# PrayagS/Seriation-in-Paleontological-Data-using-MCMC

Measured on AMD Instinct MI355X. Metric: chain-iterations/sec (100 chains, 256x512 matrix) at 1/2/4/8 MI355X, higher is better.
Workload: dtype f64

## Files before the change

### __graft_entry__.py

```python
import os
import subprocess
import sys

ROOT = os.path.dirname(os.path.abspath(__file__))
PKG = os.path.join(ROOT, "seriation-in-paleontological-data-using-mcmc_amd")


def _paths():
    for p in (PKG, os.path.join(ROOT, "tests")):
        if p not in sys.path:
            sys.path.insert(0, p)


def prewarm(test_shapes=True):
    from concurrent.futures import ThreadPoolExecutor
    _paths()
    import seriation_amd as sa
    ddir = os.path.join(ROOT, "tests", "golden", "datasets")
    paths = sorted(os.path.join(ddir, f) for f in os.listdir(ddir) if f.endswith(".txt"))

    def soft(what, fn):
        try:
            return fn()
        except sa.SrError as e:
            print("prewarm: %s skipped (%s)" % (what, e), file=sys.stderr)
            return 0

    def one(p):
        return soft(os.path.basename(p), lambda: sa.specialize(sa.Dataset.load(p, maxs=0)))

    import numpy as np

    def shape(t):
        N, M, nh, tb = t
        hard = np.zeros(N, np.uint8)
        hard[:nh] = 1
        return soft("shape %r" % (t,), lambda: sa.specialize(sa.Dataset(np.zeros((N, M), np.uint8), hard),
                                                            block_threads=tb))

    shapes = []
    if test_shapes:
        try:
            import spec_shapes
            shapes = spec_shapes.shapes()
            import test_gpu_logl_walk
            import test_gpu_sweep_tail
            shapes = sorted(set(shapes) | set(test_gpu_logl_walk.lds_shapes()) | set(test_gpu_sweep_tail.lds_shapes()))
        except ImportError:
            pass
    with ThreadPoolExecutor(max_workers=min(8, os.cpu_count() or 1)) as ex:
        out = dict(zip([os.path.basename(p) for p in paths], ex.map(one, paths)))
        out["test shapes"] = sum(bool(r) for r in ex.map(shape, shapes))
    return out


def build():
    jobs = str(min(16, os.cpu_count() or 1))
    subprocess.check_call(["make", "-s", "-j" + jobs, "-C", PKG])
    subprocess.check_call(["make", "-s", "-j" + jobs, "-C", os.path.join(ROOT, "oracle")])
    _paths()
    import seriation_amd
    seriation_amd.lib()
    prewarm()


def smoke():
    _paths()
    import numpy as np
    import oracle_ref
    import seriation_amd as sa

    if sa.lib().sr_device_count() <= 0:
        raise RuntimeError("smoke: no gfx950 device visible")
    with open(os.path.join(ROOT, "tests", "golden", "datasets", "g10s10.txt"), "rb") as fh:
        text = fh.read()
    ds = sa.Dataset.parse(text)
    seeds = [1, 2]
    summ, (ri, rd) = sa.run_chains(ds, seeds, burnin_calls=1, sample_calls=3, keep_records=True, device=0)
    for k, s in enumerate(seeds):
        o = oracle_ref.run_chain(text, s, 1, 3)
# ... 12 lines not shown
```

### include/seriation.h

```cpp
#ifndef SERIATION_H
#define SERIATION_H
#include <stddef.h>
#include <stdint.h>
#ifdef __cplusplus
extern "C" {
#endif

#define SR_OK 0
#define SR_EINVAL (-1)
#define SR_EPARSE (-2)
#define SR_EHEADER (-3)
#define SR_ENOMEM (-4)
#define SR_EDEVICE (-5)
#define SR_EUNSUPPORTED (-6)
#define SR_EIO (-7)
#define SR_EINCONSISTENT (-8)

#define SR_MAXS 2000

typedef struct {
  int32_t N, M, nh;
  uint8_t *X;
  uint8_t *hard;
} sr_dataset;
// ... 229 lines not shown
  int64_t *dist, *dist_mirror;
  int64_t scale;
  double kernel_ms;
} sr_agree_out;

int sr_agreement(const sr_dataset *ds, const int16_t *ab_pi, int32_t n_sel, int32_t count, int32_t device,
                 sr_agree_out *out);
int sr_session_agreement(sr_session *s, const int32_t *chains, int32_t n_sel, int32_t first, int32_t count,
                         sr_agree_out *out);
int sr_agreement_distances(int32_t N, int32_t n_sel, const uint32_t *pair_counts, int32_t device, int64_t *dist,
                           int64_t *dist_mirror, double *kernel_ms);
int sr_agreement_modes(int32_t n, const int64_t *dist, const int64_t *dist_mirror, int64_t scale, double threshold,
                       int32_t *mode, uint8_t *flip, int32_t *medoid, int32_t *size, int32_t *n_modes);

typedef struct {
  const uint8_t *flip;
  int64_t *order_loss;
  int64_t *limit_loss;
  uint32_t *pair_counts;
  int32_t *best;
  int32_t *state;
  int32_t central_chain, central_row;
  int64_t scale;
  double kernel_ms;
} sr_central_out;

int sr_central(const sr_dataset *ds, const int16_t *ab_pi, int32_t n_sel, int32_t count, int32_t device,
               sr_central_out *out);
int sr_session_central(sr_session *s, const int32_t *chains, int32_t n_sel, int32_t first, int32_t count,
                       sr_central_out *out);
int sr_order_loss(const sr_dataset *ds, const int16_t *ab_pi, int32_t n_sel, int32_t count, const uint8_t *flip,
                  const uint32_t *against, int32_t device, int64_t *order_loss, double *kernel_ms);

const char *sr_strerror(int code);
int sr_device_count(void);
const char *sr_version(void);

#ifdef __cplusplus
}
#endif
#endif
```

### seriation-in-paleontological-data-using-mcmc_amd/csrc/sr_device.hip

```cpp
#include <hip/hip_runtime.h>
#include <stdint.h>
#include <stdio.h>
#include <stdlib.h>
#include <string.h>
#include <unistd.h>
#include <type_traits>
#define SR_TABLES_NO_ARRAYS
#include "sr_tables.h"
#include "sr_math.h"
#include "sr_rng.h"
#include "sr_internal.h"
#include "seriation.h"

__constant__ double c_zig_y[128] = SR_ZIG_YTAB_INIT;
__constant__ unsigned int c_zig_k[128] = SR_ZIG_KTAB_INIT;
__constant__ double c_zig_w[128] = SR_ZIG_WTAB_INIT;
__constant__ uint64_t c_exp_tab[256] = SR_EXP_TAB_INIT;
__constant__ double c_log_tab[256] = SR_LOG_TAB_INIT;

#define SR_ZIGR 3.44428647676

#ifndef SR_FN
#define SR_FN 0
#endif
// ... 7 lines not shown
struct KArgs {
  int N, M, NW, nh, nchains;
  int calls, spc, save, rec_base, rec_cap;
  uint32_t *P;
  int32_t *rpi, *hp, *ab, *cnt;
  double *cdl;
  uint32_t *mt;
  uint64_t *rng, *acc;
  int16_t *rec_abpi;
  double *rec_cdl;
  unsigned long long *dbg;
  uint16_t *gpre;
  uint32_t *pkey;
  double *gck;
  double *glbuf, *gcbuf;
  int *xflag, *xbuf, *xerr;
  double *cdv, *cdx;
  double *rec_cdv;
};

#ifndef SR_CKG
#define SR_CKG 4
#endif
#ifndef SR_CERT_SHIFT
#define SR_CERT_SHIFT 0
#endif
#define SR_CERT_SCALE (1.0 / (double)(1ull << SR_CERT_SHIFT))
__device__ __forceinline__ const KArgs &kargs_late(const KArgs &A) { return A; }
#ifndef SR_TSUMS
#define SR_TSUMS 4
#endif
#ifndef SR_BATCH_MAX
#define SR_BATCH_MAX 16
#endif

struct Lay {
  size_t tab, cbuf, lbuf, mt, P, rpi0, rpi1, ht, ck, ccnt, sab, scnt, hpw, hbw, t4, t8, pre, part, tot, xs, ptab, misc, total;
};
__host__ __device__ static constexpr inline size_t sr_al16(size_t x) { return (x + 15) & ~(size_t)15; }
__host__ __device__ static constexpr inline int sr_nwm(int N) { const int nk = (N >> 5) + 1; return nk <= 9 ? 9 : (nk <= 17 ? 17 : 0); }
__host__ __device__ static constexpr inline bool sr_regwalk(int N, int M, int TB, bool gm, int nh)
{
  return !gm && TB <= 512 && M <= TB && sr_nwm(N) > 0 && nh <= 32;
}
#define T8STRIDE 514
__host__ __device__ static constexpr inline int sr_ckstride(int M, int TB) { return M >= TB ? TB : ((M + 63) & ~63); }
__host__ __device__ static constexpr inline int sr_chunk() { return 64; }
__host__ __device__ static constexpr inline Lay sr_layout(int N, int M, int NW, int TB, bool gm, int nh = 0, bool lpre = false)
{
  Lay L{};
  size_t o = 0;
  const int CH = sr_chunk(), KT = (M + CH - 1) / CH, NWV = TB / 64;
  const size_t g = gm ? 0 : 1;
  lpre = lpre && gm;
  const size_t NT = gm ? 1 : NWV;
  L.tab = o;   o = sr_al16(o + 512 * sizeof(double));
  L.cbuf = o;  o = sr_al16(o + g * 2 * KT * CH * sizeof(double));
  L.lbuf = o;  o = sr_al16(o + g * M * sizeof(double));
  L.mt = o;    o = sr_al16(o + (size_t)SR_RING * SR_MT_N * 4);
  L.P = o;     o = sr_al16(o + g * NW * M * 4);
  L.rpi0 = o;  o = sr_al16(o + (size_t)N * 4);
  L.rpi1 = o;  o = sr_al16(o + (size_t)N * 4);
  L.ht = o;    o = sr_al16(o + (gm ? 1 : (size_t)NWV) * (2 * N + 2) * 2);
  const size_t rw = sr_regwalk(N, M, TB, gm, nh) ? 1 : 0;
  L.ck = o;    o = sr_al16(o + g * (1 - rw) * ((N >> 5) + 1) * sr_ckstride(M, TB) * sizeof(double));
  L.ccnt = o;  o = sr_al16(o + (size_t)2 * KT * 4);
// ... 1529 lines not shown
    const int s_lo = (xa - hcnt[xa]) - ri, s_hi = (xb - hcnt[xb]) - ri;
    auto hard_ones = [&](int lo, int hi, int &cnt) -> int {
      if (hi < lo) { cnt = 0; return 0; }
      const int kl = hcnt[lo], kh = hcnt[hi + 1];
      cnt = kh - kl;
      if (hbx) {
        int o = 0;
        for (int w = lo >> 5; w <= (hi >> 5); ++w) o += __popc(Pm[w * M] & hbx[w] & range_mask(w, lo, hi));
        return o;
      }
      constexpr int HB = 8 * (int)sizeof(HM);
      const HM km = ((kh >= HB) ? ~(HM)0 : (((HM)1 << kh) - (HM)1)) & ~((kl >= HB) ? ~(HM)0 : (((HM)1 << kl) - (HM)1));
      return (int)__popcll((uint64_t)(hbm & km));
    };
    const int wlo = max(a, i), whi = min(b - 1, j);
    const int sizeW = max(0, whi - wlo + 1);
    int onesI = 0, sizeI = 0;
    const int onesW = (whi >= wlo) ? col_pre(prem, Pm, M, whi + 1, PS) - col_pre(prem, Pm, M, wlo, PS) : 0;
    if (s_lo < s_hi) {
      const int pl = nhall[ri + q.Kn - s_hi], ph = nhall[ri + q.Kn - s_lo - 1];
      int hc;
      const int ho = hard_ones(pl, ph, hc);
      onesI = col_pre(prem, Pm, M, ph + 1, PS) - col_pre(prem, Pm, M, pl, PS) - ho;
      sizeI = s_hi - s_lo;
    }
    {
      int hc;
      const int ho = hard_ones(max(na, i), min(nb - 1, j), hc);
      onesI += ho;
      sizeI += hc;
    }
    dt1 = onesI - onesW;
    dt0 = (sizeW - onesW) - (sizeI - onesI);
  }
}


template <bool GM, bool SP, typename XSync>
__device__ __forceinline__ double sr_exact_delta(int kind, Prop q, CD K, const int32_t *sab, const uint32_t *P, const uint16_t *pre,
                                              int M, int N, int KT, int olo, int ohi,
                                              int hl, int nh, const int16_t *hcnt, const int16_t *nhall, const uint32_t *hbx,
                                              double *cb, int *cc, double *xs,
                                              int lane, int wave, int TB, XSync &&xsync, const double *kv = nullptr,
                                              const double *kx = nullptr, int PS = 0)
{
  constexpr int CH = sr_chunk();
  for (int m0 = olo + wave * CH; m0 < ohi; m0 += TB) {
    const int ch = m0 / CH, m = m0 + lane;
    int dt0 = 0, dt1 = 0;
    if (m < M)
      taxon_dt(kind, q, sab[m], sab[M + m], P + m, pre + m, M, kind == PK_PI3 ? hard_bits_col<uint64_t>(P + m, M, hl, nh) : 0ull,
               hcnt, nhall, dt0, dt1, hbx, PS);
    CD Km = K;
    if (kv && m < M) { Km.c = kv[m]; Km.d = kv[M + m]; Km.cc = kx[m]; Km.dd = kx[M + m]; }
    const double tv = (m < M) ? qval(dt0, -dt0, dt1, -dt1, Km) : 0.0;
    const uint64_t msk = __ballot(tv != 0.0);
    const int pos = __builtin_amdgcn_mbcnt_hi((uint32_t)(msk >> 32), __builtin_amdgcn_mbcnt_lo((uint32_t)msk, 0u));
    if (tv != 0.0) { if constexpr (SP) xst(cb + ch * CH + pos, tv); else cb[ch * CH + pos] = tv; }
    if (lane == 0) { if constexpr (SP) xst(cc + ch, (int)__popcll(msk)); else cc[ch] = __popcll(msk); }
  }
  if constexpr (SP) xsync(); else __syncthreads();
  if constexpr (GM) return exact_sum_gm<SP>(cb, cc, KT, lane, CH);
  else return exact_sum_wave(cb, cc, KT, xs, lane, CH);
}

#define SR_RNG_SLACK 1024
// ... 581 lines not shown
          }
          if ((p0 > 0 || (!GM && pend == 1)) && !(ROLE && predrawn)) {
            int delta = tvalid ? (int)((rblk - tblk) * SR_MT_N + roff) - (int)toff : 0;
            if (!tvalid || delta < 0 || delta + 5 * (16 - p0) + 5 > 128) {
              delta = 0;
              tblk = rblk; toff = roff; tvalid = true;
#if defined(SR_STAMPS) && !defined(SR_STAMP_FINE)
              if (tid == 0) misc[42] += 1;
#endif
#pragma unroll
              for (int h = 0; h < 2; ++h)
                ptab_fill(ptab, ring, base, avail, lane + 64 * h, -1, N, nh, hcnt, nhall, mdN, mdN1, md2, mdH, mdH1);
              wsync();
            }
            FST(15);
            prop_scan(ptab, ring, base, avail, delta, p0, lane, vpk, vkr, vuw, vnd, voff, pend, off);
          }
          for (int p = pend; p < 16; ++p) {
            if (p0 == 0 && p == 1) break;
            if (p > p0) break;
            if (!scalar_one(p)) break;
          }
          pend = __builtin_amdgcn_readfirstlane(pend);
#if defined(SR_STAMPS) && !defined(SR_STAMP_FINE)
          if (tid == 0 && pend > p0) { misc[40] += 1; misc[41] += (unsigned long long)(pend - p0); }
#endif
          FST(2);
          STAMP_D(4);
          if (pend == p0) {
            rng_ensure(R, min(avail + 256, (SR_RING - 1) * SR_MT_N - (SR_MT_N - 1)), tid, TB);
            tvalid = false;
            continue;
          }
          auto load_prop = [&](int p) -> Prop {
            Prop q;
            const uint32_t pk = (uint32_t)__builtin_amdgcn_readlane(vpk, p);
            q.i = (int)(pk & 4095u);
            q.j = (int)((pk >> 12) & 4095u);
            q.ii = min(q.i, q.j); q.jj = max(q.i, q.j);
            q.inc1 = (int)((pk >> 24) & 1u); q.inc2 = (int)((pk >> 25) & 1u);
            const uint32_t kr = (uint32_t)__builtin_amdgcn_readlane(vkr, p);
            q.Kn = (int)(kr & 0xffffu);
            q.r0 = (int)(kr >> 16);
            return q;
          };
          auto vetoed = [&](int p) -> bool { return ((uint32_t)__builtin_amdgcn_readlane(vpk, p) >> 26) & 1u; };

          int *pw = part + (bpar * 16) * NWV * 8;
          const bool pack = N < 512;
          const bool one = NWM > 0 || (SP && TB == 1024) || (SP && ohi - olo <= TB) || M <= TB;
          int a1 = 0, b1 = 0;
          const HM hb1 = hbc;
          constexpr bool ALLOWN = !SP && SR_FM > 0 && SR_FM >= TB;
          const bool own = ALLOWN || mt < ohi;
          if (one && own) { a1 = sab[mt]; b1 = sab[M + mt]; }
          FST(13);
#if defined(SR_STAMP_DRAWS)
          STAMP(5);
#elif defined(SR_STAMP_GIBBS)
          STAMP(6);
#else
          STAMP(3);
#endif
          if (one) {
            int d0s[16], d1s[16];
#pragma unroll
            for (int sI = 0; sI < 16; ++sI) {
              d0s[sI] = 0; d1s[sI] = 0;
              if (sI >= p0 && sI < pend && !vetoed(sI)) {
                const Prop q = load_prop(sI);
                int dt0 = 0, dt1 = 0;
                if (own) taxon_dt(prop_kind(sI), q, a1, b1, P + mt, pre + mt, M, hb1, hcnt, nhall, dt0, dt1, hbx, PS);
                d0s[sI] = dt0; d1s[sI] = dt1;
              }
            }
            FST(3);
            if (SR_TSUMS && !GM && pack && pend - p0 >= SR_TSUMS) {
              uint32_t u[32];
#pragma unroll
              for (int sI = 0; sI < 16; ++sI) {
                u[sI] = (uint32_t)(d0s[sI] + N) | ((uint32_t)(d1s[sI] + N) << 16);
                u[16 + sI] = (uint32_t)((d0s[sI] | d1s[sI]) != 0) | ((uint32_t)(d0s[sI] != 0) << 16);
              }
              const uint32_t v = wave_sum32_t(u, lane);
              const int sl = (((lane >> 1) & 1) << 3) | (((lane >> 2) & 1) << 2) | (((lane >> 3) & 1) << 1) | ((lane >> 4) & 1);
              const uint32_t pk = (uint32_t)__builtin_amdgcn_ds_bpermute(sl << 2, vpk);
              if (lane < 32) {
                int w0, w1;
                if (!(lane & 1)) { w0 = (int)(v & 0xffffu) - 64 * N; w1 = (int)(v >> 16) - 64 * N; }
                else {
                  const int any = (int)(v & 0xffffu), c0 = (int)(v >> 16);
                  const int pi = (int)(pk & 4095u), pj = (int)((pk >> 12) & 4095u);
                  const bool p1 = sl > 0 && (sl - 1) % 3 == 0;
                  w0 = p1 ? c0 : any * 2 * (max(pi, pj) - min(pi, pj) + 1);
                  w1 = p1 ? any - c0 : w0;
                }
                int *o = pw + (sl * NWV + wave) * 8 + 2 * (lane & 1);
                o[0] = w0; o[1] = w1;
              }
            } else if (SR_TSUMS && !pack && !GM && pend - p0 >= SR_TSUMS) {
              uint32_t u[32];
#pragma unroll
              for (int sI = 0; sI < 16; ++sI) { u[sI] = (uint32_t)d0s[sI]; u[16 + sI] = (uint32_t)d1s[sI]; }
              const int vx = (int)wave_sum32_t(u, lane);
#pragma unroll
              for (int sI = 0; sI < 16; ++sI) { u[sI] = (uint32_t)abs(d0s[sI]); u[16 + sI] = (uint32_t)abs(d1s[sI]); }
              const int vy = (int)wave_sum32_t(u, lane);
// ... 1196 lines not shown
                                                                int n, int *out)
{
  __shared__ double tabs[512];
  for (int i = threadIdx.x; i < 256; i += blockDim.x) {
    ((uint64_t *)tabs)[i] = c_exp_tab[i];
    tabs[256 + i] = c_log_tab[i];
  }
  __syncthreads();
  sr_mtab tb;
  tb.exp_tab = (const uint64_t *)tabs; tb.log_tab = tabs + 256;
  const int m = blockIdx.x * blockDim.x + threadIdx.x;
  if (m >= n) return;
  CD K;
  K.c = cd[2 * m]; K.d = cd[2 * m + 1];
  K.cc = sr_log_m(1. - sr_exp_m(K.c, &tb), &tb);
  K.dd = sr_log_m(1. - sr_exp_m(K.d, &tb), &tb);
  K.ec = 0.0;
  const double aC = __builtin_fabs(K.cc) + __builtin_fabs(K.d), aD = __builtin_fabs(K.dd) + __builtin_fabs(K.c);
  double Sp, Ebp;
  int Knz;
  const int cls = pc_classify(sums[4 * m], sums[4 * m + 1], sums[4 * m + 2], sums[4 * m + 3], K, aC, aD, uw[m], Sp,
                              Ebp, Knz);
  int res = 0;
  if (cls != 0) {
    bool accept, udrawn = false, have_exact;
    double dl;
    const double u = (double)uw[m] / 4294967296.0;
    if (!pc_resolve(Sp, Ebp, cls, Knz, u, tb, accept, udrawn, have_exact, dl)) res = 3;
    else res = accept ? (udrawn ? 2 : 1) : 0;
  }
  out[m] = res;
}

extern "C" __attribute__((visibility("default"))) int sr_device_selftest_gibbs(int device, int mode, int N, int ncases,
                                                                              const uint32_t *P, const uint16_t *pre,
                                                                              const double *cd, const int *o, const int *L,
                                                                              const int *rev, const double *u, int *out,
                                                                              unsigned long long *fb)
{
  const int NW = (N + 31) >> 5;
  if (ncases <= 0 || ncases % 64 || N < 1 || N > 4095 || mode < 0 || mode > 3 || (mode == 0 && NW > 9) ||
      (mode == 1 && NW > 17))
    return -1;
  for (int m = 0; m < ncases; ++m)
    if (o[m] < 0 || o[m] > L[m] || L[m] > N) return -1;
  HIPCHK(hipSetDevice(device));
  const size_t C = (size_t)ncases;
  void *b[11] = {};
  const size_t sz[11] = {NW * C * 4, (NW + 1) * C * 2, C / 64 * 2 * 8, C * 4, C * 4, C * 4, C * 8, C * 5 * 4, C * 8,
                         (NW + 2) * C * 8, 0};
  int rc = 0;
  for (int k = 0; k < 10 && !rc; ++k) rc = hipMalloc(&b[k], sz[k]) != hipSuccess;
  const void *src[7] = {P, pre, cd, o, L, rev, u};
  for (int k = 0; k < 7 && !rc; ++k) rc = hipMemcpy(b[k], src[k], sz[k], hipMemcpyHostToDevice) != hipSuccess;
  if (!rc) rc = hipMemset(b[8], 0, sz[8]) != hipSuccess;
  if (!rc) {
    const dim3 g(ncases / 64), t(64);
    const uint32_t *dP = (const uint32_t *)b[0];
    const uint16_t *dpre = (const uint16_t *)b[1];
    const double *dcd = (const double *)b[2], *du = (const double *)b[6];
    const int *dO = (const int *)b[3], *dL = (const int *)b[4], *dR = (const int *)b[5];
    int *dout = (int *)b[7];
    unsigned long long *dfb = (unsigned long long *)b[8];
    double *dck = (double *)b[9];
    if (mode == 0) hipLaunchKernelGGL(sr_gibbs_selftest_kernel<0>, g, t, 0, 0, dP, dpre, N, ncases, dcd, dO, dL, dR, du, dout, dfb, dck);
    else if (mode == 1) hipLaunchKernelGGL(sr_gibbs_selftest_kernel<1>, g, t, 0, 0, dP, dpre, N, ncases, dcd, dO, dL, dR, du, dout, dfb, dck);
    else if (mode == 2) hipLaunchKernelGGL(sr_gibbs_selftest_kernel<2>, g, t, 0, 0, dP, dpre, N, ncases, dcd, dO, dL, dR, du, dout, dfb, dck);
    else hipLaunchKernelGGL(sr_gibbs_selftest_kernel<3>, g, t, 0, 0, dP, dpre, N, ncases, dcd, dO, dL, dR, du, dout, dfb, dck);
    rc = hipGetLastError() != hipSuccess || hipDeviceSynchronize() != hipSuccess;
  }
  if (!rc) rc = hipMemcpy(out, b[7], sz[7], hipMemcpyDeviceToHost) != hipSuccess;
  if (!rc) rc = hipMemcpy(fb, b[8], sz[8], hipMemcpyDeviceToHost) != hipSuccess;
  for (int k = 0; k < 10; ++k) (void)hipFree(b[k]);
  return rc ? -2 : 0;
}

extern "C" __attribute__((visibility("default"))) int sr_device_selftest_decide(int device, int ncases, const int *sums,
                                                                               const double *cd, const uint32_t *uw,
                                                                               int *out)
{
  if (ncases <= 0) return -1;
  HIPCHK(hipSetDevice(device));
  const size_t C = (size_t)ncases;
  void *b[4] = {};
  const size_t sz[4] = {C * 16, C * 16, C * 4, C * 4};
  int rc = 0;
  for (int k = 0; k < 4 && !rc; ++k) rc = hipMalloc(&b[k], sz[k]) != hipSuccess;
  const void *src[3] = {sums, cd, uw};
  for (int k = 0; k < 3 && !rc; ++k) rc = hipMemcpy(b[k], src[k], sz[k], hipMemcpyHostToDevice) != hipSuccess;
  if (!rc) {
    hipLaunchKernelGGL(sr_decide_selftest_kernel, dim3((ncases + 63) / 64), dim3(64), 0, 0, (const int *)b[0],
                       (const double *)b[1], (const uint32_t *)b[2], ncases, (int *)b[3]);
    rc = hipGetLastError() != hipSuccess || hipDeviceSynchronize() != hipSuccess;
  }
  if (!rc) rc = hipMemcpy(out, b[3], sz[3], hipMemcpyDeviceToHost) != hipSuccess;
  for (int k = 0; k < 4; ++k) (void)hipFree(b[k]);
  return rc ? -2 : 0;
}
#endif
```

### seriation-in-paleontological-data-using-mcmc_amd/seriation_amd/_lib.py

```python
import ctypes
import os

PKG_DIR = os.path.dirname(os.path.dirname(os.path.abspath(__file__)))
LIB_PATH = os.environ.get("SERIATION_LIB") or os.path.join(PKG_DIR, "build", "libseriation.so")

SR_OK = 0
SR_EINVAL = -1
SR_EPARSE = -2
SR_EHEADER = -3
SR_ENOMEM = -4
SR_EDEVICE = -5
SR_EUNSUPPORTED = -6
SR_EIO = -7
SR_EINCONSISTENT = -8
SR_MAXS = 2000
SR_F_NO_CHECK = 1
SR_F_HBM_COLUMNS = 2
SR_F_LDS_COLUMNS = 4
SR_F_DEBUG_CHECK = 8
SR_F_DEBUG_PRINT = 16
SR_F_RNG_PHILOX = 32
SR_F_DIAG = 64
SR_F_GENERIC_KERNEL = 128

# ... 126 lines not shown


class sr_central_out(ctypes.Structure):
    _fields_ = [("flip", ctypes.POINTER(ctypes.c_uint8)),
                ("order_loss", ctypes.POINTER(ctypes.c_int64)), ("limit_loss", ctypes.POINTER(ctypes.c_int64)),
                ("pair_counts", ctypes.POINTER(ctypes.c_uint32)),
                ("best", ctypes.POINTER(ctypes.c_int32)), ("state", ctypes.POINTER(ctypes.c_int32)),
                ("central_chain", ctypes.c_int32), ("central_row", ctypes.c_int32),
                ("scale", ctypes.c_int64),
                ("kernel_ms", ctypes.c_double)]


SINK_FN = ctypes.CFUNCTYPE(ctypes.c_int, ctypes.c_void_p, ctypes.c_int32, ctypes.c_int32,
                           ctypes.POINTER(sr_record))

PUBLIC_SYMBOLS = [
    "sr_parse_dataset", "sr_load_dataset", "sr_free_dataset", "sr_save_dataset_bin", "sr_load_dataset_bin",
    "sr_default_opts", "sr_rng_env_setup",
    "sr_run_chains", "sr_run_to_dirs", "sr_run_chains_multi", "sr_run_to_dirs_multi", "sr_session_create", "sr_session_set_stream",
    "sr_session_run", "sr_session_sync", "sr_session_records", "sr_session_record_capacity",
    "sr_session_fetch_records", "sr_session_reset_records", "sr_session_fetch_chain_records", "sr_session_copy_chain_records", "sr_session_summaries",
    "sr_session_fetch_cd_vectors", "sr_session_manycd", "sr_session_state_cd",
    "sr_session_state",
    "sr_session_accept_counts", "sr_session_fallback_counts", "sr_session_debug_flagged", "sr_session_last_kernel_ms", "sr_session_block_threads", "sr_session_variant", "sr_session_specialized",
    "sr_session_checkpoint", "sr_session_restore",
    "sr_session_destroy", "sr_specialize", "sr_posterior", "sr_session_posterior",
    "sr_diagnostics", "sr_session_diagnostics", "sr_diag_reduce", "sr_marginals", "sr_session_marginals",
    "sr_relations", "sr_session_relations", "sr_waic", "sr_session_waic", "sr_waic_reduce",
    "sr_loo", "sr_session_loo", "sr_loo_reduce", "sr_loo_tail", "sr_loo_tail_len",
    "sr_ppc", "sr_session_ppc", "sr_occupancy", "sr_session_occupancy",
    "sr_placement", "sr_session_placement",
    "sr_agreement", "sr_session_agreement", "sr_agreement_distances", "sr_agreement_modes",
    "sr_central", "sr_session_central", "sr_order_loss",
    "sr_strerror", "sr_device_count", "sr_version",
]

_LIB = None


def _lib():
    global _LIB
    if _LIB is not None:
        return _LIB
    if not os.path.exists(LIB_PATH):
        raise ImportError("libseriation.so not built (%s); run __graft_entry__.build()" % LIB_PATH)
    L = ctypes.CDLL(LIB_PATH)
    P = ctypes.POINTER
    c_int, c_i32, c_void_p, c_double = ctypes.c_int, ctypes.c_int32, ctypes.c_void_p, ctypes.c_double
    sig = {
        "sr_parse_dataset": (c_int, [ctypes.c_char_p, ctypes.c_size_t, c_i32, P(sr_dataset)]),
        "sr_load_dataset": (c_int, [ctypes.c_char_p, c_i32, P(sr_dataset)]),
        "sr_free_dataset": (None, [P(sr_dataset)]),
        "sr_save_dataset_bin": (c_int, [P(sr_dataset), ctypes.c_char_p]),
        "sr_load_dataset_bin": (c_int, [ctypes.c_char_p, P(sr_dataset)]),
        "sr_default_opts": (None, [P(sr_run_opts)]),
        "sr_rng_env_setup": (c_int, [P(ctypes.c_uint64), c_i32]),
        "sr_run_chains": (c_int, [P(sr_dataset), P(sr_chain_spec), c_i32, P(sr_run_opts), SINK_FN,
                                  c_void_p, P(sr_chain_summary)]),
        "sr_run_to_dirs": (c_int, [P(sr_dataset), P(sr_chain_spec), c_i32, P(sr_run_opts),
                                   ctypes.c_char_p, P(sr_chain_summary)]),
        "sr_run_chains_multi": (c_int, [P(sr_dataset), P(sr_chain_spec), c_i32, P(sr_run_opts), P(c_i32), c_i32,
                                        SINK_FN, c_void_p, P(sr_chain_summary)]),
        "sr_run_to_dirs_multi": (c_int, [P(sr_dataset), P(sr_chain_spec), c_i32, P(sr_run_opts), P(c_i32), c_i32,
                                         ctypes.c_char_p, P(sr_chain_summary)]),
        "sr_session_create": (c_int, [P(sr_dataset), P(sr_chain_spec), c_i32, P(sr_run_opts), P(c_void_p)]),
        "sr_session_set_stream": (c_int, [c_void_p, c_void_p]),
# ... 28 lines not shown
        "sr_diag_reduce": (c_int, [c_i32, c_i32, c_i32, c_i32, P(ctypes.c_int64), P(ctypes.c_int64), P(ctypes.c_int64),
                                   P(ctypes.c_int64), P(c_double), P(c_double), P(c_double), P(c_i32)]),
        "sr_marginals": (c_int, [P(sr_dataset), P(ctypes.c_int16), c_i32, c_i32, c_i32, P(sr_marg_out)]),
        "sr_session_marginals": (c_int, [c_void_p, P(c_i32), c_i32, c_i32, c_i32, P(sr_marg_out)]),
        "sr_relations": (c_int, [P(sr_dataset), P(ctypes.c_int16), c_i32, c_i32, c_i32, P(sr_rel_out)]),
        "sr_session_relations": (c_int, [c_void_p, P(c_i32), c_i32, c_i32, c_i32, P(sr_rel_out)]),
        "sr_waic": (c_int, [P(sr_dataset), P(ctypes.c_int16), P(c_double), c_i32, c_i32, c_i32, c_i32, P(sr_waic_out)]),
        "sr_session_waic": (c_int, [c_void_p, P(c_i32), c_i32, c_i32, c_i32, P(sr_waic_out)]),
        "sr_waic_reduce": (c_int, [c_i32, c_i32, P(c_double), P(c_double), P(sr_waic_out)]),
        "sr_loo": (c_int, [P(sr_dataset), P(ctypes.c_int16), P(c_double), c_i32, c_i32, c_i32, c_i32, P(sr_loo_out)]),
        "sr_session_loo": (c_int, [c_void_p, P(c_i32), c_i32, c_i32, c_i32, P(sr_loo_out)]),
        "sr_loo_reduce": (c_int, [c_i32, c_i32, P(c_double), P(c_double), P(c_double), P(sr_loo_out)]),
        "sr_loo_tail": (c_int, [ctypes.c_int64, c_i32, P(c_double), c_double, c_double, P(c_double), P(c_double)]),
        "sr_loo_tail_len": (c_i32, [ctypes.c_int64]),
        "sr_ppc": (c_int, [P(sr_dataset), P(ctypes.c_int16), P(c_double), c_i32, c_i32, c_i32, ctypes.c_uint64, c_i32,
                           c_i32, P(sr_ppc_out)]),
        "sr_session_ppc": (c_int, [c_void_p, P(c_i32), c_i32, c_i32, c_i32, ctypes.c_uint64, c_i32, P(sr_ppc_out)]),
        "sr_occupancy": (c_int, [P(sr_dataset), P(ctypes.c_int16), c_i32, c_i32, c_i32, P(sr_occ_out)]),
        "sr_session_occupancy": (c_int, [c_void_p, P(c_i32), c_i32, c_i32, c_i32, P(sr_occ_out)]),
        "sr_placement": (c_int, [P(sr_dataset), P(ctypes.c_int16), P(c_double), c_i32, c_i32, c_i32, P(ctypes.c_uint8),
                                 c_i32, c_i32, P(sr_place_out)]),
        "sr_session_placement": (c_int, [c_void_p, P(c_i32), c_i32, c_i32, c_i32, P(ctypes.c_uint8), c_i32,
                                         P(sr_place_out)]),
        "sr_agreement": (c_int, [P(sr_dataset), P(ctypes.c_int16), c_i32, c_i32, c_i32, P(sr_agree_out)]),
        "sr_session_agreement": (c_int, [c_void_p, P(c_i32), c_i32, c_i32, c_i32, P(sr_agree_out)]),
        "sr_agreement_distances": (c_int, [c_i32, c_i32, P(ctypes.c_uint32), c_i32, P(ctypes.c_int64),
                                           P(ctypes.c_int64), P(c_double)]),
        "sr_agreement_modes": (c_int, [c_i32, P(ctypes.c_int64), P(ctypes.c_int64), ctypes.c_int64, c_double,
                                       P(c_i32), P(ctypes.c_uint8), P(c_i32), P(c_i32), P(c_i32)]),
        "sr_central": (c_int, [P(sr_dataset), P(ctypes.c_int16), c_i32, c_i32, c_i32, P(sr_central_out)]),
        "sr_session_central": (c_int, [c_void_p, P(c_i32), c_i32, c_i32, c_i32, P(sr_central_out)]),
        "sr_order_loss": (c_int, [P(sr_dataset), P(ctypes.c_int16), c_i32, c_i32, P(ctypes.c_uint8),
                                  P(ctypes.c_uint32), c_i32, P(ctypes.c_int64), P(c_double)]),
        "sr_strerror": (ctypes.c_char_p, [c_int]),
        "sr_device_count": (c_int, []),
        "sr_version": (ctypes.c_char_p, []),
        "sr_host_exp_log": (None, [P(c_double), ctypes.c_long, P(c_double), P(c_double)]),
        "sr_host_run_add": (c_double, [c_double, c_double, ctypes.c_long]),
        "sr_host_run_sub": (ctypes.c_long, [P(c_double), c_double, ctypes.c_long]),
        "sr_host_philox": (None, [P(ctypes.c_uint32), P(ctypes.c_uint32), P(ctypes.c_uint32)]),
        "sr_host_mt_untemper": (None, [P(ctypes.c_uint32), ctypes.c_long, P(ctypes.c_uint32), P(ctypes.c_uint32)]),
        "sr_host_mt_block": (c_int, [ctypes.c_ulong, c_int, P(ctypes.c_uint32), P(ctypes.c_uint32)]),
        "sr_host_initial_checkpoint": (c_int, [P(sr_dataset), P(sr_chain_spec), c_i32, ctypes.c_char_p]),
        "sr_host_init_chain": (c_int, [P(sr_dataset), ctypes.c_uint64, P(c_i32), P(c_i32), P(c_i32),
                                       P(c_double), P(ctypes.c_uint64)]),
        "sr_spec_cache_path": (c_int, [c_int, c_int, c_int, c_int, ctypes.c_char_p, ctypes.c_size_t]),
        "sr_session_debug_counters": (c_int, [c_void_p, P(ctypes.c_ulonglong)]),
        "sr_session_spec_embedded": (c_i32, [c_void_p]),
        "sr_spec_is_embedded": (c_int, [c_int, c_int, c_int, c_int]),
        "sr_device_selftest_math": (c_int, [c_int, P(c_double), ctypes.c_long, P(c_double), P(c_double)]),
        "sr_device_selftest_udiv": (c_int, [c_int, P(ctypes.c_uint32), P(ctypes.c_uint32), ctypes.c_long,
                                            P(ctypes.c_uint32)]),
    }
    for name, (res, args) in sig.items():
        if not hasattr(L, name):
            continue
        fn = getattr(L, name)
        fn.restype = res
        fn.argtypes = args
    _LIB = L
    return L


def lib():
    return _lib()
```

Baseline: 5.417 million.

## Stage per-batch taxon term loads to overlap memory latency across proposals

Replaces the per-proposal taxon_dt loop with a staged batch_terms routine. It first issues all column-prefix and hard-count loads for up to 16 proposals, then computes the terms in later phases separated by sched_barrier. The aim is to hide global and LDS load latency by keeping many independent loads in flight, where before each proposal waited on its own serial load chain. The cost is much higher register pressure from the per-slot staging arrays, which could lower occupancy. A selftest kernel and entry point are added to check the new path against the old one.

```diff
diff --git a/__graft_entry__.py b/__graft_entry__.py
--- a/__graft_entry__.py
+++ b/__graft_entry__.py
@@ -45,7 +45,9 @@
             shapes = spec_shapes.shapes()
             import test_gpu_logl_walk
             import test_gpu_sweep_tail
-            shapes = sorted(set(shapes) | set(test_gpu_logl_walk.lds_shapes()) | set(test_gpu_sweep_tail.lds_shapes()))
+            import test_gpu_terms_chains
+            shapes = sorted(set(shapes) | set(test_gpu_logl_walk.lds_shapes()) | set(test_gpu_sweep_tail.lds_shapes()) |
+                            set(test_gpu_terms_chains.lds_shapes()))
         except ImportError:
             pass
     with ThreadPoolExecutor(max_workers=min(8, os.cpu_count() or 1)) as ex:
diff --git a/include/seriation.h b/include/seriation.h
--- a/include/seriation.h
+++ b/include/seriation.h
@@ -285,6 +285,9 @@
 int sr_order_loss(const sr_dataset *ds, const int16_t *ab_pi, int32_t n_sel, int32_t count, const uint8_t *flip,
                   const uint32_t *against, int32_t device, int64_t *order_loss, double *kernel_ms);
 
+int sr_device_selftest_terms(int device, int mode, int N, int M, int nh, const int32_t *hard_pos, const uint32_t *P,
+                             int ncases, const int32_t *ab, const int32_t *recs, int32_t *out);
+
 const char *sr_strerror(int code);
 int sr_device_count(void);
 const char *sr_version(void);
diff --git a/seriation-in-paleontological-data-using-mcmc_amd/csrc/sr_device.hip b/seriation-in-paleontological-data-using-mcmc_amd/csrc/sr_device.hip
--- a/seriation-in-paleontological-data-using-mcmc_amd/csrc/sr_device.hip
+++ b/seriation-in-paleontological-data-using-mcmc_amd/csrc/sr_device.hip
@@ -63,6 +63,12 @@
 #endif
 #ifndef SR_BATCH_MAX
 #define SR_BATCH_MAX 16
+#endif
+#ifndef SR_TERMS_STAGED
+#define SR_TERMS_STAGED 1
+#endif
+#ifndef SR_TERMS_MINP3
+#define SR_TERMS_MINP3 0
 #endif
 
 struct Lay {
@@ -1658,6 +1664,160 @@
     }
     dt1 = onesI - onesW;
     dt0 = (sizeW - onesW) - (sizeI - onesI);
+  }
+}
+
+__device__ __forceinline__ int batch_p3(int p0, int pend) { return (pend + 2) / 3 - (max(p0, 1) + 2) / 3; }
+
+__device__ __forceinline__ Prop prop_unpack(int vpk, int vkr, int p)
+{
+  Prop q;
+  const uint32_t pk = (uint32_t)__builtin_amdgcn_readlane(vpk, p);
+  q.i = (int)(pk & 4095u);
+  q.j = (int)((pk >> 12) & 4095u);
+  q.ii = min(q.i, q.j); q.jj = max(q.i, q.j);
+  q.inc1 = (int)((pk >> 24) & 1u); q.inc2 = (int)((pk >> 25) & 1u);
+  const uint32_t kr = (uint32_t)__builtin_amdgcn_readlane(vkr, p);
+  q.Kn = (int)(kr & 0xffffu);
+  q.r0 = (int)(kr >> 16);
+  return q;
+}
+
+__device__ __forceinline__ void col_pre_issue(const uint16_t *prem, const uint32_t *Pm, int M, int NW, int x, int PS,
+                                              uint32_t &word, uint16_t &pv)
+{
+  const int w = x >> 5;
+  word = Pm[min(w, NW - 1) * M];
+  pv = prem[w * (PS ? PS : M)];
+}
+__device__ __forceinline__ int col_pre_done(uint32_t word, uint16_t pv, int x) { return (int)pv + __popc(word & ((1u << (x & 31)) - 1u)); }
+
+template <typename HM>
+__device__ __forceinline__ void batch_terms(int vpk, int vkr, int p0, int pend, int a, int b, HM hbm, const uint32_t *Pm,
+                                            const uint16_t *prem, int M, int NW, int PS, const int16_t *hcnt,
+                                            const int16_t *nhall, int (&d0s)[16], int (&d1s)[16])
+{
+  auto act = [&](int s) -> bool {
+    return s >= p0 && s < pend && !(((uint32_t)__builtin_amdgcn_readlane(vpk, s) >> 26) & 1u);
+  };
+  auto hard_mask = [&](int kl, int kh) -> int {
+    constexpr int HB = 8 * (int)sizeof(HM);
+    const HM km = ((kh >= HB) ? ~(HM)0 : (((HM)1 << kh) - (HM)1)) & ~((kl >= HB) ? ~(HM)0 : (((HM)1 << kl) - (HM)1));
+    return (int)__popcll((uint64_t)(hbm & km));
+  };
+  auto mirror = [&](const Prop &q, int &na, int &nb) {
+    const int ain = ininterval(a, q.i, q.j + 1, q.inc1, q.inc2);
+    const int bin = ininterval(b, q.i, q.j + 1, q.inc1, q.inc2);
+    const int t = q.i + q.j + 1;
+    na = ain ? (bin ? t - b : t - a) : a;
+    nb = bin ? (ain ? t - a : t - b) : b;
+  };
+  uint32_t w0[16], w1[16], w2[16];
+  uint16_t u0[16], u1[16], u2[16];
+  int16_t h0[16], h1[16], h2[16], h3[16];
+  int v0[16], v1[16], v2[16];
+#pragma unroll
+  for (int s = 0; s < 16; ++s) {
+    d0s[s] = 0; d1s[s] = 0;
+    w0[s] = w1[s] = w2[s] = 0u;
+    u0[s] = u1[s] = u2[s] = 0;
+    h0[s] = h1[s] = h2[s] = h3[s] = 0;
+    v0[s] = v1[s] = v2[s] = 0;
+  }
+#pragma unroll
+  for (int s = 0; s < 16; ++s) {
+    if (!act(s)) continue;
+    const Prop q = prop_unpack(vpk, vkr, s);
+    const int kind = prop_kind(s);
+    if (kind == PK_PI1) {
+      w0[s] = Pm[(q.i >> 5) * M];
+    } else if (kind != PK_PI3) {
+      const int ain = ininterval(a, q.i, q.j + 1, q.inc1, q.inc2);
+      const int sp = ain ? a : b;
+      col_pre_issue(prem, Pm, M, NW, q.i, PS, w0[s], u0[s]);
+      col_pre_issue(prem, Pm, M, NW, sp, PS, w1[s], u1[s]);
+      col_pre_issue(prem, Pm, M, NW, q.j + 1, PS, w2[s], u2[s]);
+    } else {
+      int na, nb;
+      mirror(q, na, nb);
+      const int xa = min(max(na, q.i), q.j + 1), xb = min(max(nb, q.i), q.j + 1);
+      h0[s] = hcnt[xa];
+      h1[s] = hcnt[xb];
+      v1[s] = na; v2[s] = nb;
+    }
+  }
+  __builtin_amdgcn_sched_barrier(0);
+#pragma unroll
+  for (int s = 0; s < 16; ++s) {
+    if (!act(s)) continue;
+    const Prop q = prop_unpack(vpk, vkr, s);
+    const int kind = prop_kind(s);
+    const int i = q.i, j = q.j;
+    if (kind == PK_PI1) {
+      const int v = (w0[s] >> (i & 31)) & 1;
+      const int up = i < j ? 1 : 0, L = q.ii + up, span = q.jj - q.ii;
+      const int ain = (uint32_t)(a - L) <= (uint32_t)span, bin = (uint32_t)(b - L) <= (uint32_t)span;
+      const int sgn = up ? ain - bin : bin - ain;
+      d1s[s] = v ? sgn : 0;
+      d0s[s] = v ? 0 : -sgn;
+    } else if (kind != PK_PI3) {
+      const int ain = ininterval(a, i, j + 1, q.inc1, q.inc2);
+      const int bin = ininterval(b, i, j + 1, q.inc1, q.inc2);
+      const int sp = ain ? a : b;
+      const int c0 = col_pre_done(w0[s], u0[s], i), c1 = col_pre_done(w1[s], u1[s], sp), c2 = col_pre_done(w2[s], u2[s], j + 1);
+      const int O1 = c1 - c0, O2 = c2 - c1;
+      const int Z1 = (sp - i) - O1, Z2 = (j + 1 - sp) - O2;
+      const int e1 = ain ? O1 - O2 : O2 - O1, e0 = ain ? Z2 - Z1 : Z1 - Z2;
+      d1s[s] = ain != bin ? e1 : 0;
+      d0s[s] = ain != bin ? e0 : 0;
+    } else {
+      const int ri = q.r0;
+      const int na = v1[s], nb = v2[s];
+      const int xa = min(max(na, i), j + 1), xb = min(max(nb, i), j + 1);
+      const int s_lo = (xa - (int)h0[s]) - ri, s_hi = (xb - (int)h1[s]) - ri;
+      const bool ok = s_lo < s_hi;
+      h0[s] = nhall[ok ? ri + q.Kn - s_hi : 0];
+      h1[s] = nhall[ok ? ri + q.Kn - s_lo - 1 : 0];
+      col_pre_issue(prem, Pm, M, NW, min(b, j + 1), PS, w0[s], u0[s]);
+      col_pre_issue(prem, Pm, M, NW, max(a, i), PS, w1[s], u1[s]);
+      h2[s] = hcnt[max(na, i)];
+      h3[s] = hcnt[min(nb, j + 1)];
+      v0[s] = s_hi - s_lo;
+    }
+  }
+  __builtin_amdgcn_sched_barrier(0);
+#pragma unroll
+  for (int s = 0; s < 16; ++s) {
+    if (prop_kind(s) != PK_PI3 || !act(s)) continue;
+    const Prop q = prop_unpack(vpk, vkr, s);
+    const int i = q.i, j = q.j;
+    const bool ok = v0[s] > 0;
+    const int pl = ok ? (int)h0[s] : 0, ph = ok ? (int)h1[s] : 0;
+    const int wlo = max(a, i), wh1 = min(b, j + 1);
+    const int onesW = wh1 > wlo ? col_pre_done(w0[s], u0[s], wh1) - col_pre_done(w1[s], u1[s], wlo) : 0;
+    const int sizeW = max(0, wh1 - wlo);
+    const int lo2 = max(v1[s], i), e2 = min(v2[s], j + 1);
+    const int kl2 = e2 > lo2 ? (int)h2[s] : 0, kh2 = e2 > lo2 ? (int)h3[s] : 0;
+    const int ho2 = hard_mask(kl2, kh2), hc2 = kh2 - kl2;
+    h0[s] = hcnt[pl];
+    h1[s] = hcnt[ph + 1];
+    col_pre_issue(prem, Pm, M, NW, ph + 1, PS, w0[s], u0[s]);
+    col_pre_issue(prem, Pm, M, NW, pl, PS, w1[s], u1[s]);
+    d1s[s] = ho2 - onesW;
+    d0s[s] = (sizeW - onesW) - (hc2 - ho2);
+    v1[s] = pl; v2[s] = ph;
+  }
+  __builtin_amdgcn_sched_barrier(0);
+#pragma unroll
+  for (int s = 0; s < 16; ++s) {
+    if (prop_kind(s) != PK_PI3 || !act(s)) continue;
+    const bool ok = v0[s] > 0;
+    const int pl = v1[s], ph = v2[s];
+    const int kl = ph < pl ? 0 : (int)h0[s], kh = ph < pl ? 0 : (int)h1[s];
+    const int oI = col_pre_done(w0[s], u0[s], ph + 1) - col_pre_done(w1[s], u1[s], pl) - hard_mask(kl, kh);
+    const int onesI = ok ? oI : 0, sizeI = ok ? v0[s] : 0;
+    d1s[s] += onesI;
+    d0s[s] -= sizeI - onesI;
   }
 }
 
@@ -2305,18 +2465,7 @@
             tvalid = false;
             continue;
           }
-          auto load_prop = [&](int p) -> Prop {
-            Prop q;
-            const uint32_t pk = (uint32_t)__builtin_amdgcn_readlane(vpk, p);
-            q.i = (int)(pk & 4095u);
-            q.j = (int)((pk >> 12) & 4095u);
-            q.ii = min(q.i, q.j); q.jj = max(q.i, q.j);
-            q.inc1 = (int)((pk >> 24) & 1u); q.inc2 = (int)((pk >> 25) & 1u);
-            const uint32_t kr = (uint32_t)__builtin_amdgcn_readlane(vkr, p);
-            q.Kn = (int)(kr & 0xffffu);
-            q.r0 = (int)(kr >> 16);
-            return q;
-          };
+          auto load_prop = [&](int p) -> Prop { return prop_unpack(vpk, vkr, p); };
           auto vetoed = [&](int p) -> bool { return ((uint32_t)__builtin_amdgcn_readlane(vpk, p) >> 26) & 1u; };
 
           int *pw = part + (bpar * 16) * NWV * 8;
@@ -2337,6 +2486,14 @@
 #endif
           if (one) {
             int d0s[16], d1s[16];
+            bool staged = false;
+            if constexpr (SR_TERMS_STAGED && SR_FN > 0 && TB <= 512 && !GM && !MCD)
+              staged = hbx == nullptr && (SR_TERMS_MINP3 == 0 || batch_p3(p0, pend) >= SR_TERMS_MINP3);
+            if (staged) {
+#pragma unroll
+              for (int sI = 0; sI < 16; ++sI) { d0s[sI] = 0; d1s[sI] = 0; }
+              if (own) batch_terms<HM>(vpk, vkr, p0, pend, a1, b1, hb1, P + mt, pre + mt, M, NW, PS, hcnt, nhall, d0s, d1s);
+            } else {
 #pragma unroll
             for (int sI = 0; sI < 16; ++sI) {
               d0s[sI] = 0; d1s[sI] = 0;
@@ -2346,6 +2503,7 @@
                 if (own) taxon_dt(prop_kind(sI), q, a1, b1, P + mt, pre + mt, M, hb1, hcnt, nhall, dt0, dt1, hbx, PS);
                 d0s[sI] = dt0; d1s[sI] = dt1;
               }
+            }
             }
             FST(3);
             if (SR_TSUMS && !GM && pack && pend - p0 >= SR_TSUMS) {
@@ -3608,6 +3766,53 @@
   out[m] = res;
 }
 
+template <int MODE>
+__global__ void __launch_bounds__(64) sr_terms_selftest_kernel(const uint32_t *P, uint16_t *pre, int N, int M, int nh,
+                                                               const int *hpos, const int *ab, const int *recs, int *out)
+{
+  using HM = typename std::conditional<MODE == 2, uint32_t, uint64_t>::type;
+  __shared__ int hp[4096];
+  __shared__ uint32_t hbw[128];
+  __shared__ int16_t hcnt[4096], nhall[4096];
+  const int lane = threadIdx.x, m = blockIdx.x * 64 + lane, cs = blockIdx.y;
+  const int NW = (N + 31) >> 5;
+  for (int k = lane; k < nh; k += 64) hp[k] = hpos[k];
+  wsync();
+  build_hard_tables(hp, nh, N, NW, hbw, hcnt, nhall, lane);
+  const bool own = m < M;
+  const int mc = own ? m : 0;
+  pre += (size_t)cs * (NW + 1) * M;
+  if (own) col_pre_build(pre + m, P + m, M, NW);
+  const int hl0 = (lane < nh) ? hp[lane] : 0;
+  const HM hbc = own ? hard_bits_col<HM>(P + m, M, hl0, nh) : (HM)0;
+  const uint32_t *hbx = nh > SR_NHMAX ? hbw : nullptr;
+  const int *rc = recs + 34 * cs;
+  const int vpk = lane < 16 ? rc[lane] : 1 << 26, vkr = lane < 16 ? rc[16 + lane] : 0;
+  const int p0 = rc[32], pend = rc[33];
+  const int a1 = own ? ab[(size_t)cs * 2 * M + m] : 0, b1 = own ? ab[(size_t)cs * 2 * M + M + m] : 0;
+  int d0s[16], d1s[16];
+#pragma unroll
+  for (int sI = 0; sI < 16; ++sI) { d0s[sI] = 0; d1s[sI] = 0; }
+  if constexpr (MODE == 0) {
+#pragma unroll
+    for (int sI = 0; sI < 16; ++sI) {
+      if (sI >= p0 && sI < pend && !(((uint32_t)__builtin_amdgcn_readlane(vpk, sI) >> 26) & 1u)) {
+        const Prop q = prop_unpack(vpk, vkr, sI);
+        int dt0 = 0, dt1 = 0;
+        if (own) taxon_dt(prop_kind(sI), q, a1, b1, P + mc, pre + mc, M, hbc, hcnt, nhall, dt0, dt1, hbx);
+        d0s[sI] = dt0; d1s[sI] = dt1;
+      }
+    }
+  } else {
+    if (own) batch_terms<HM>(vpk, vkr, p0, pend, a1, b1, hbc, P + mc, pre + mc, M, NW, 0, hcnt, nhall, d0s, d1s);
+  }
+  if (own) {
+    int *o = out + ((size_t)cs * M + m) * 32;
+#pragma unroll
+    for (int sI = 0; sI < 16; ++sI) { o[2 * sI] = d0s[sI]; o[2 * sI + 1] = d1s[sI]; }
+  }
+}
+
 extern "C" __attribute__((visibility("default"))) int sr_device_selftest_gibbs(int device, int mode, int N, int ncases,
                                                                               const uint32_t *P, const uint16_t *pre,
                                                                               const double *cd, const int *o, const int *L,
@@ -3673,4 +3878,64 @@
   for (int k = 0; k < 4; ++k) (void)hipFree(b[k]);
   return rc ? -2 : 0;
 }
+
+extern "C" __attribute__((visibility("default"))) int sr_device_selftest_terms(int device, int mode, int N, int M, int nh,
+                                                                              const int32_t *hard_pos, const uint32_t *P,
+                                                                              int ncases, const int32_t *ab,
+                                                                              const int32_t *recs, int32_t *out)
+{
+  if (mode < 0 || mode > 2 || N < 2 || N > 4095 || M < 1 || M > (1 << 20) || nh < 0 || nh > N || ncases < 1 ||
+      ncases > 65535 || !P || !ab || !recs || !out || (nh > 0 && !hard_pos))
+    return -1;
+  if ((mode == 1 && nh > SR_NHMAX) || (mode == 2 && nh > 32)) return -1;
+  int hc[4097] = {0};
+  for (int k = 0; k < nh; ++k) {
+    if (hard_pos[k] < 0 || hard_pos[k] >= N || (k > 0 && hard_pos[k] <= hard_pos[k - 1])) return -1;
+    hc[(size_t)hard_pos[k] + 1] = 1;
+  }
+  for (int x = 1; x <= N; ++x) hc[x] += hc[x - 1];
+  for (int cs = 0; cs < ncases; ++cs) {
+    const int32_t *r = recs + 34 * (size_t)cs;
+    for (size_t k = 0; k < 2 * (size_t)M; ++k)
+      if (ab[(size_t)cs * 2 * M + k] < 0 || ab[(size_t)cs * 2 * M + k] > N) return -1;
+    if (r[32] < 0 || r[32] > r[33] || r[33] > 16) return -1;
+    for (int s = r[32]; s < r[33]; ++s) {
+      const uint32_t pk = (uint32_t)r[s], kr = (uint32_t)r[16 + s];
+      if (pk >> 27) return -1;
+      if ((pk >> 26) & 1u) continue;
+      const int i = (int)(pk & 4095u), j = (int)((pk >> 12) & 4095u), kind = s == 0 ? 0 : 1 + (s - 1) % 3;
+      if (i >= N || j >= N) return -1;
+      if (kind != 1 && i >= j) return -1;
+      if (kind == 0 && j != i + 1) return -1;
+      if (kind == 3) {
+        if (hc[i + 1] != hc[i] || hc[j + 1] != hc[j]) return -1;
+        const int ri = i - hc[i], rj = j - hc[j];
+        if ((int)(kr >> 16) != ri || (int)(kr & 0xffffu) != rj - ri + 1) return -1;
+      }
+    }
+  }
+  HIPCHK(hipSetDevice(device));
+  const size_t NW = (size_t)(N + 31) >> 5, C = (size_t)ncases;
+  void *b[6] = {};
+  const size_t sz[6] = {NW * M * 4, (size_t)(nh > 0 ? nh : 1) * 4, C * 2 * M * 4, C * 34 * 4, C * (NW + 1) * M * 2, C * M * 32 * 4};
+  int rc = 0;
+  for (int k = 0; k < 6 && !rc; ++k) rc = hipMalloc(&b[k], sz[k]) != hipSuccess;
+  const void *src[4] = {P, hard_pos, ab, recs};
+  for (int k = 0; k < 4 && !rc; ++k)
+    if (k != 1 || nh > 0) rc = hipMemcpy(b[k], src[k], k == 1 ? (size_t)nh * 4 : sz[k], hipMemcpyHostToDevice) != hipSuccess;
+  if (!rc) {
+    const dim3 g((unsigned)((M + 63) / 64), (unsigned)ncases), t(64);
+    const uint32_t *dP = (const uint32_t *)b[0];
+    const int *dh = (const int *)b[1], *dab = (const int *)b[2], *dr = (const int *)b[3];
+    uint16_t *dpre = (uint16_t *)b[4];
+    int *dout = (int *)b[5];
+    if (mode == 0) hipLaunchKernelGGL(sr_terms_selftest_kernel<0>, g, t, 0, 0, dP, dpre, N, M, nh, dh, dab, dr, dout);
+    else if (mode == 1) hipLaunchKernelGGL(sr_terms_selftest_kernel<1>, g, t, 0, 0, dP, dpre, N, M, nh, dh, dab, dr, dout);
+    else hipLaunchKernelGGL(sr_terms_selftest_kernel<2>, g, t, 0, 0, dP, dpre, N, M, nh, dh, dab, dr, dout);
+    rc = hipGetLastError() != hipSuccess || hipDeviceSynchronize() != hipSuccess;
+  }
+  if (!rc) rc = hipMemcpy(out, b[5], sz[5], hipMemcpyDeviceToHost) != hipSuccess;
+  for (int k = 0; k < 6; ++k) (void)hipFree(b[k]);
+  return rc ? -2 : 0;
+}
 #endif
diff --git a/seriation-in-paleontological-data-using-mcmc_amd/seriation_amd/_lib.py b/seriation-in-paleontological-data-using-mcmc_amd/seriation_amd/_lib.py
--- a/seriation-in-paleontological-data-using-mcmc_amd/seriation_amd/_lib.py
+++ b/seriation-in-paleontological-data-using-mcmc_amd/seriation_amd/_lib.py
@@ -182,6 +182,7 @@
     "sr_placement", "sr_session_placement",
     "sr_agreement", "sr_session_agreement", "sr_agreement_distances", "sr_agreement_modes",
     "sr_central", "sr_session_central", "sr_order_loss",
+    "sr_device_selftest_terms",
     "sr_strerror", "sr_device_count", "sr_version",
 ]
 
@@ -276,6 +277,8 @@
         "sr_session_central": (c_int, [c_void_p, P(c_i32), c_i32, c_i32, c_i32, P(sr_central_out)]),
         "sr_order_loss": (c_int, [P(sr_dataset), P(ctypes.c_int16), c_i32, c_i32, P(ctypes.c_uint8),
                                   P(ctypes.c_uint32), c_i32, P(ctypes.c_int64), P(c_double)]),
+        "sr_device_selftest_terms": (c_int, [c_int, c_int, c_int, c_int, c_int, P(c_i32), P(ctypes.c_uint32), c_int,
+                                             P(c_i32), P(c_i32), P(c_i32)]),
         "sr_strerror": (ctypes.c_char_p, [c_int]),
         "sr_device_count": (c_int, []),
         "sr_version": (ctypes.c_char_p, []),
```

After: 5.234 million. -3.4%, worse.
